# facebookresearch/ProcedureVRL

Measured on AMD Instinct MI355X. Metric: training clips/sec (8f x 224^2, ViT-B TimeSformer), higher is better.
Workload: dtype f16; 1 GPU; TimeSformer ViT-B 8x224^2, 32 clips/GPU, K=9871 step logits, top-5 KL + all-gather InfoNCE, fwd+bwd+AdamW (BASELINE configs[1]; configs[2] at 8 GPUs); clips_per_gpu=32, global_batch=32, parallelism=dp1

## Files before the change

procedurevrl_amd/csrc/attn_bwd_fused.hip:

```cpp
#include "attn_stream.h"
#include "../../include/pvrl.h"

namespace {

constexpr int FB_PRIO7 = 3, FB_PRIO46 = 1;
constexpr int FB_DS = FB_ROWS * 64;
constexpr int FB_Q = 0, FB_D = FB_TILE, FB_K = 2 * FB_TILE, FB_S = 4 * FB_TILE, FB_INIT = 4 * FB_TILE + 2 * FB_DS;
constexpr int FB_O = FB_INIT + 4 * FB_ROWS * 4;
constexpr int FB_LSE = FB_O + 3 * 4096;
constexpr int FB_LDS = FB_LSE + 3 * 256;

struct FbCopy { int o, r0, col; };
__device__ __forceinline__ FbCopy fb_copy_init(int o, int lane) {
  FbCopy cp;
  cp.o = o;
  const int j = o & 3;
  const int band = lane >> 5;
  cp.r0 = 8 * j + 4 * band + ((lane >> 1) & 3);
  const int cb = ((lane >> 3) & 3) ^ band, half = (lane & 1) ^ (j & 1);
  cp.col = 16 * cb + 8 * half;
  if (o >= 12) { cp.r0 = lane & 31; cp.col = 0; }
  return cp;
}
__device__ __forceinline__ void fb_slot_op(const AttnArgs& p, const FbItem& it, int jb, const FbCopy& cp, int rs, int S, unsigned ldsbase) {
  const int rc = min(32 * jb + cp.r0, S - 1);
  const unsigned rowi = rc == 0 ? (unsigned)it.sr.base0 : (unsigned)it.sr.base1 + (unsigned)(rc - 1) * (unsigned)it.sr.stride;
  if (cp.o >= 12) {
    const float* lp = p.lse + ((long)it.seq * p.H + it.h) * S + rc;
    asm volatile("s_mov_b32 m0, %1\n\tglobal_load_lds_dword %0, off" :: "v"(lp), "s"(ldsbase + FB_LSE + rs * 256) : "memory", "m0");
    return;
  }
  const int j = cp.o & 3, typ = cp.o >> 2;
  const int hc = it.h * 64 + cp.col;
  if (typ == 0) {
    glds16_raw_v(p.qkv + (unsigned long long)rowi * (unsigned)p.ld + hc, ldsbase + FB_Q + (4 * jb + j) * 1024);
  } else {
    const op_t* tok = typ == 1 ? p.d_o : p.ofw;
    const op_t* cls = typ == 1 ? p.d_o_cls : p.ofw_cls;
    const op_t* a = tok + (unsigned long long)rowi * (unsigned)p.ldo;
    const op_t* b = cls + (long)it.seq * p.ldo;
    const op_t* src = (p.mp.mode == 1 && rc == 0) ? b : a;
    glds16_raw_v(src + hc, ldsbase + (typ == 1 ? FB_D + (4 * jb + j) * 1024 : FB_O + (4 * rs + j) * 1024));
  }
}
__device__ __forceinline__ void fb_finalize_quarter(const char* smem, int jb, int rs, int qtr, int S, float scale, int lane, float* si) {
  const int pidx = 64 * qtr + lane;
  const int r = pidx >> 3, c8 = (pidx & 7) * 8, row = 32 * jb + r;
  const u32x4 d = *reinterpret_cast<const u32x4*>(smem + FB_D + fb_off(row, c8));
  const u32x4 o = *reinterpret_cast<const u32x4*>(smem + FB_O + rs * 4096 + fb_off(r, c8));
  const float l = reinterpret_cast<const float*>(smem + FB_LSE)[rs * 64 + r];
  float dsum = 0.f;
#pragma unroll
  for (int e = 0; e < 4; ++e) {
    float a0, a1, b0, b1;
    op_unpack2(d[e], a0, a1);
    op_unpack2(o[e], b0, b1);
    dsum = fmaf(a0, b0, dsum);
    dsum = fmaf(a1, b1, dsum);
  }
  dsum = fb_sum8(dsum);
  if ((pidx & 7) == 0) {
    const bool keep = row < S;
    si[row] = keep ? -l * (1.0f / scale) : -INFINITY;
    si[FB_ROWS + row] = keep ? -dsum * scale : 0.f;
  }
}
__device__ __forceinline__ void fb_prime_pair(const AttnArgs& p, const FbItem& it, int pidx, int S, float* si) {
  const int row = pidx >> 3, c8 = (pidx & 7) * 8;
  const int rc = min(row, S - 1);
  const u32x4 d = *reinterpret_cast<const u32x4*>(fb_tok(p.d_o, p.d_o_cls, p.ldo, p, it, rc) + it.h * 64 + c8);
  const u32x4 o = *reinterpret_cast<const u32x4*>(fb_tok(p.ofw, p.ofw_cls, p.ldo, p, it, rc) + it.h * 64 + c8);
  const float l = p.lse[((long)it.seq * p.H + it.h) * S + rc];
  float dsum = 0.f;
#pragma unroll
  for (int e = 0; e < 4; ++e) {
    float a0, a1, b0, b1;
    op_unpack2(d[e], a0, a1);
    op_unpack2(o[e], b0, b1);
    dsum = fmaf(a0, b0, dsum);
    dsum = fmaf(a1, b1, dsum);
  }
  dsum = fb_sum8(dsum);
  if ((pidx & 7) == 0 && row < FB_ROWS) {
    const bool keep = row < S;
    si[row] = keep ? -l / p.scale : -INFINITY;
    si[FB_ROWS + row] = keep ? -dsum * p.scale : 0.f;
  }
}

template <int NQB>
__device__ __forceinline__ void dq_block(const AttnArgs& p, const FbItem& it, const char* Kb, const char* dsr, int nqb, int S,
                                         int jb, int lane) {
  const int g = lane >> 5, hi = (lane >> 4) & 1, i = lane & 15;
  f32x16 acc[2];
#pragma unroll
  for (int dh = 0; dh < 2; ++dh)
#pragma unroll
    for (int r = 0; r < 16; ++r) acc[dh][r] = 0.f;
  const int inb = (i >> 2) * 32 + ((8 * (i & 3)) ^ (16 * g)) + g * 1024;
  const int a0 = inb + hi * 128, a1 = inb + 512 + (hi ^ 1) * 128;
  const int b0 = (2 * g) * 256 + hi * 128 + (i >> 2) * 32 + (((i & 3) ^ (2 * g)) * 8);
  const int b1 = (2 * g + 1) * 256 + hi * 128 + (i >> 2) * 32 + (((i & 3) ^ (2 * g + 1)) * 8);
  auto load = [&](int ks, opx8& bf, opx8* af) {
    bf = tr_frag8(dsr + ks * 1024, b0, b1);
#pragma unroll
    for (int dh = 0; dh < 2; ++dh) af[dh] = tr_frag8(Kb + ks * 2048 + dh * 256, a0, a1);
  };
  if constexpr (NQB > 0) {
    opx8 bf[3], af[3][2];
    load(0, bf[0], af[0]);
    load(1, bf[1], af[1]);
#pragma unroll
    for (int ks = 0; ks < 2 * NQB; ++ks) {
      if (ks + 2 < 2 * NQB) load(ks + 2, bf[(ks + 2) % 3], af[(ks + 2) % 3]);
      __builtin_amdgcn_sched_barrier(0);
#pragma unroll
      for (int dh = 0; dh < 2; ++dh) {
        acc[dh] = MFMA_32x32x16(af[ks % 3][dh], bf[ks % 3], acc[dh], 0, 0, 0);
      }
      __builtin_amdgcn_sched_barrier(0);
    }
  } else {
#pragma unroll 1
    for (int ks = 0; ks < 2 * nqb; ++ks) {
      opx8 bf, af[2];
      load(ks, bf, af);
#pragma unroll
      for (int dh = 0; dh < 2; ++dh) acc[dh] = MFMA_32x32x16(af[dh], bf, acc[dh], 0, 0, 0);
    }
  }
  char* st = const_cast<char*>(dsr);
  {
    const int q = lane & 31;
#pragma unroll
    for (int dh = 0; dh < 2; ++dh)
#pragma unroll
      for (int j = 0; j < 4; ++j) {
        opx4 ov;
#pragma unroll
        for (int r = 0; r < 4; ++r) ov[r] = (op_t)acc[dh][4 * j + r];
        *reinterpret_cast<opx4*>(st + q * 128 + (((4 * dh + j) ^ (q & 7)) * 16) + 8 * g) = ov;
      }
  }
#pragma unroll
  for (int t = 0; t < 4; ++t) {
    const int idx = lane + 64 * t;
    const int r = idx >> 3, ch = idx & 7;
    const u32x4 v = *reinterpret_cast<const u32x4*>(st + r * 128 + ((ch ^ (r & 7)) * 16));
    const int query = 32 * jb + r;
    if (query < S) *reinterpret_cast<u32x4*>(fb_tok(p.dqkv, p.dqkv_cls, p.ldd, p, it, query) + it.h * 64 + ch * 8) = v;
  }
}

template <int NQB>
__global__ __launch_bounds__(512, 2) void attn_bwd_fused_kernel(AttnArgs p, int nvb) {
  __shared__ __attribute__((aligned(16))) char smem[FB_LDS];
  const int tid = threadIdx.x, lane = tid & 63;
  const int wave = __builtin_amdgcn_readfirstlane(tid >> 6);
  const int S = p.mp.S;
  const int nqb = NQB > 0 ? NQB : (S + 31) >> 5;
  const int HD = p.H * PVRL_HEAD_DIM;
  const int n = lane & 31, g = lane >> 5;
  const bool keywave = wave < nqb;
  const float c = p.scale * 1.4426950408889634f;
  const unsigned ldsbase = __builtin_amdgcn_readfirstlane(lds_addr(smem));

  FbItem cur, nxt;
  int vcur = -1;
  int vnxt = fb_next(p, blockIdx.x, gridDim.x, nvb, nxt);
  int par = 0;
  int nit = -1;
  if (vnxt < 0) return;

  {
    float* si = reinterpret_cast<float*>(smem + FB_INIT) + (par ^ 1) * 2 * FB_ROWS;
#pragma unroll
    for (int t = 0; t < 4; ++t) fb_prime_pair(p, nxt, tid + 512 * t, S, si);
  }

  if (wave == 7) {
    __builtin_amdgcn_s_setprio(FB_PRIO7);
    while (true) {
      if (vcur >= 0) {
#pragma unroll 1
        for (int jb = 0; jb < nqb; ++jb) {
          FB_BARRIER();
          dq_block<NQB>(p, cur, smem + FB_K + par * FB_TILE, smem + FB_S + (jb & 1) * FB_DS, nqb, S, jb, lane);
        }
      }
      if (vnxt < 0) break;
      FB_BARRIER();
      par ^= 1; ++nit;
      cur = nxt; vcur = vnxt;
      vnxt = fb_next(p, vcur + gridDim.x, gridDim.x, nvb, nxt);
    }
    return;
  }

  const int rbl = n >> 2, b0 = rbl & 1, b1 = (rbl >> 1) & 1;
  const int rowbase = rbl * 512 + (n & 3) * 32 + ((16 * g) ^ (16 * b1));
  const int e0 = rowbase + b0 * 128, e1 = rowbase + (1 - b0) * 128;
  const int i16 = lane & 15, hi = (lane >> 4) & 1;
  const int trb = g * 512 + (hi ^ g) * 128 + (i16 >> 2) * 32;
  const int tr0 = trb + 8 * (i16 & 3), tr1 = trb + 1024 + ((8 * (i16 & 3)) ^ 16);
  const int kbl = rbl & 3;
  const int dsw0 = (8 * wave + rbl) * 256 + (n & 3) * 32;
  const bool lastkw = wave == nqb - 1 && (S & 31) != 0;
  const float keepf = (32 * wave + n) < S ? 1.f : 0.f;
  const int ncp = wave < 4 ? 3 : (wave == 4 ? 1 : 0);
  const FbCopy cp1 = fb_copy_init(wave < 4 ? wave : 12, lane), cp2 = fb_copy_init(4 + (wave & 3), lane), cp3 = fb_copy_init(8 + (wave & 3), lane);
  if (wave >= 4) __builtin_amdgcn_s_setprio(FB_PRIO46);
  opx8 kf[4], vf[4];
  f32x16 dk[2], dvv[2];
  while (true) {
    opx8 vfn[4];
    if (vnxt >= 0) {
#pragma unroll
      for (int j = 0; j < 4; ++j) {
        const int k = wave + 7 * j;
        int rc, col;
        fb_piece_src(k, lane, S, rc, col);
        glds16_raw_v(p.qkv + row_of(nxt.sr, rc) * p.ld + HD + nxt.h * 64 + col, ldsbase + FB_K + (par ^ 1) * FB_TILE + k * 1024);
      }
      const int key = min(32 * wave + n, S - 1);
      const op_t* vp = p.qkv + row_of(nxt.sr, key) * p.ld + 2 * HD + nxt.h * 64 + 8 * g;
#pragma unroll
      for (int s = 0; s < 4; ++s) vfn[s] = *reinterpret_cast<const opx8*>(vp + 16 * s);
    }

    if (vcur >= 0) {
#pragma unroll
      for (int dh = 0; dh < 2; ++dh)
#pragma unroll
        for (int r = 0; r < 16; ++r) { dk[dh][r] = 0.f; dvv[dh][r] = 0.f; }
      const float* sinit = reinterpret_cast<const float*>(smem + FB_INIT) + par * 2 * FB_ROWS;
      const float* dinit = sinit + FB_ROWS;
#pragma unroll 1
      for (int jb = 0; jb < nqb; ++jb) {
        char* dsj = smem + FB_S + (jb & 1) * FB_DS;
        if (wave < 4) {
          if (jb >= 3) {
            if (vnxt >= 0)
              fb_finalize_quarter(smem, jb - 3, (nqb * nit + jb - 3) % 3, wave, S, p.scale, lane,
                                  reinterpret_cast<float*>(smem + FB_INIT) + (par ^ 1) * 2 * FB_ROWS);
          } else if (jb >= 1 && nit >= 1) {
            fb_finalize_quarter(smem, nqb - 3 + jb, (nqb * (nit - 1) + nqb - 3 + jb) % 3, wave, S, p.scale, lane,
                                reinterpret_cast<float*>(smem + FB_INIT) + par * 2 * FB_ROWS);
          }
        }
        if (keywave) {
          const char* Qj = smem + FB_Q + jb * 4096;
          const char* Dj = smem + FB_D + jb * 4096;
          f32x16 sacc, dacc;
#pragma unroll
          for (int j = 0; j < 4; ++j) {
            const f32x4 a = *reinterpret_cast<const f32x4*>(sinit + 32 * jb + 8 * j + 4 * g);
            const f32x4 b = *reinterpret_cast<const f32x4*>(dinit + 32 * jb + 8 * j + 4 * g);
#pragma unroll
            for (int r = 0; r < 4; ++r) { sacc[4 * j + r] = a[r]; dacc[4 * j + r] = b[r]; }
          }
#pragma unroll
          for (int s = 0; s < 4; ++s) {
            const opx8 qa = *reinterpret_cast<const opx8*>(Qj + ((s & 1) ? e1 : e0) + 256 * (s >> 1));
            sacc = MFMA_32x32x16(qa, kf[s], sacc, 0, 0, 0);
          }
#pragma unroll
          for (int s = 0; s < 4; ++s) {
            const opx8 da = *reinterpret_cast<const opx8*>(Dj + ((s & 1) ? e1 : e0) + 256 * (s >> 1));
            dacc = MFMA_32x32x16(da, vf[s], dacc, 0, 0, 0);
          }
          if (vnxt >= 0 && jb >= 1) {
            const int rs = (nqb * nit + jb - 1) % 3;
            if (ncp >= 1) fb_slot_op(p, nxt, jb - 1, cp1, rs, S, ldsbase);
            if (ncp >= 3) { fb_slot_op(p, nxt, jb - 1, cp2, rs, S, ldsbase); fb_slot_op(p, nxt, jb - 1, cp3, rs, S, ldsbase); }
          }
          opx8 pf[2], sf[2];
#pragma unroll
          for (int r = 0; r < 16; ++r) {
            const float pr = __builtin_amdgcn_exp2f(c * sacc[r]);
            float dsv = pr * dacc[r];
            if (lastkw) dsv *= keepf;
            pf[r >> 3][r & 7] = (op_t)pr;
            sf[r >> 3][r & 7] = (op_t)dsv;
          }
#pragma unroll
          for (int t = 0; t < 2; ++t)
#pragma unroll
            for (int dh = 0; dh < 2; ++dh) {
              const opx8 ad = tr_frag8(Dj + t * 2048 + dh * 256, tr0, tr1);
              dvv[dh] = MFMA_32x32x16(ad, pf[t], dvv[dh], 0, 0, 0);
              const opx8 aq = tr_frag8(Qj + t * 2048 + dh * 256, tr0, tr1);
              dk[dh] = MFMA_32x32x16(aq, sf[t], dk[dh], 0, 0, 0);
            }
#pragma unroll
          for (int j = 0; j < 4; ++j) {
            const int slot = 2 * (j & 1) + g;
            opx4 w;
#pragma unroll
            for (int r = 0; r < 4; ++r) w[r] = sf[j >> 1][4 * (j & 1) + r];
            *reinterpret_cast<opx4*>(dsj + dsw0 + (j >> 1) * 128 + ((slot ^ kbl) * 8)) = w;
          }
        }
        if (!keywave && vnxt >= 0 && jb >= 1) {
          const int rs = (nqb * nit + jb - 1) % 3;
          if (ncp >= 1) fb_slot_op(p, nxt, jb - 1, cp1, rs, S, ldsbase);
          if (ncp >= 3) { fb_slot_op(p, nxt, jb - 1, cp2, rs, S, ldsbase); fb_slot_op(p, nxt, jb - 1, cp3, rs, S, ldsbase); }
        }
        if (ncp >= 3) asm volatile("s_waitcnt vmcnt(3)" ::: "memory");
        else if (ncp >= 1) asm volatile("s_waitcnt vmcnt(1)" ::: "memory");
        else asm volatile("s_waitcnt vmcnt(0)" ::: "memory");
        FB_BARRIER();
      }
      if (wave < 4 && vnxt >= 0)
        fb_finalize_quarter(smem, nqb - 3, (nqb * nit + nqb - 3) % 3, wave, S, p.scale, lane,
                            reinterpret_cast<float*>(smem + FB_INIT) + (par ^ 1) * 2 * FB_ROWS);
      if (vnxt >= 0) {
        const int rs = (nqb * nit + nqb - 1) % 3;
        if (ncp >= 1) fb_slot_op(p, nxt, nqb - 1, cp1, rs, S, ldsbase);
        if (ncp >= 3) { fb_slot_op(p, nxt, nqb - 1, cp2, rs, S, ldsbase); fb_slot_op(p, nxt, nqb - 1, cp3, rs, S, ldsbase); }
      }
    } else {
#pragma unroll 1
      for (int q = 0; q < 8; ++q) fb_slot_op(p, nxt, wave, fb_copy_init(q, lane), 0, S, ldsbase);
      asm volatile("s_waitcnt vmcnt(0)" ::: "memory");
    }

    if (vcur >= 0 && keywave) {
      char* st = smem + FB_S + (nqb & 1) * FB_DS + wave * 2048;
#pragma unroll
      for (int rnd = 0; rnd < 4; ++rnd) {
        const int half = rnd & 1;
        const f32x16* src = (rnd >> 1) ? dvv : dk;
        if ((n >> 4) == half) {
          const int q = n & 15;
#pragma unroll
          for (int dh = 0; dh < 2; ++dh)
#pragma unroll
            for (int j = 0; j < 4; ++j) {
              opx4 ov;
#pragma unroll
              for (int r = 0; r < 4; ++r) ov[r] = (op_t)src[dh][4 * j + r];
              *reinterpret_cast<opx4*>(st + q * 128 + (((4 * dh + j) ^ (q & 7)) * 16) + 8 * g) = ov;
            }
        }
        asm volatile("" ::: "memory");
#pragma unroll
        for (int t = 0; t < 2; ++t) {
          const int idx = lane + 64 * t;
          const int r = idx >> 3, ch = idx & 7;
          const u32x4 v = *reinterpret_cast<const u32x4*>(st + r * 128 + ((ch ^ (r & 7)) * 16));
          const int key = 32 * wave + 16 * half + r;
          if (key < S)
            *reinterpret_cast<u32x4*>(fb_tok(p.dqkv, p.dqkv_cls, p.ldd, p, cur, key) + ((rnd >> 1) ? 2 * HD : HD) + cur.h * 64 + ch * 8) = v;
        }
      }
    }
    if (vnxt < 0) break;
    FB_BARRIER();
    par ^= 1; ++nit;
    cur = nxt; vcur = vnxt;
    vnxt = fb_next(p, vcur + gridDim.x, gridDim.x, nvb, nxt);
    {
      const char* Kc = smem + FB_K + par * FB_TILE + wave * 4096;
#pragma unroll
      for (int s = 0; s < 4; ++s) {
        kf[s] = *reinterpret_cast<const opx8*>(Kc + ((s & 1) ? e1 : e0) + 256 * (s >> 1));
#pragma unroll
        for (int e = 0; e < 8; ++e) vf[s][e] = (op_t)((float)vfn[s][e] * p.scale);
      }
    }
  }
}

}

bool pvrl_attn_bwd_fused_ok(const AttnArgs& p) {
  if (p.causal || p.kpm) return false;
  if (p.mp.S <= 96 || p.mp.S > FB_ROWS) return false;
  if ((long)p.nseq * p.mp.S >= (1L << 31)) return false;
  if ((p.ldd % 8) || (p.ldo % 8)) return false;
  int e = 0;
  const float m = frexpf(p.scale, &e);
  return m == 0.5f;
}

int pvrl_attn_bwd_fused_launch(const AttnArgs& p, hipStream_t s) {
  const int cus = 8 * pvrl_compute_cus_per_xcd();
  const int nvb = 8 * ((p.nseq + 7) / 8) * p.H;
  const int grid = nvb < cus ? nvb : cus;
  if (p.mp.S > 192) hipLaunchKernelGGL(attn_bwd_fused_kernel<7>, dim3(grid), dim3(512), 0, s, p, nvb);
  else hipLaunchKernelGGL(attn_bwd_fused_kernel<0>, dim3(grid), dim3(512), 0, s, p, nvb);
  PVRL_LAUNCH_CHECK();
  return PVRL_OK;
}
```

procedurevrl_amd/csrc/attn_mfma.hip:

```cpp
#include "attn_common.h"
#include "../../include/pvrl.h"

bool pvrl_attn_bwd_fused_ok(const AttnArgs& p);
int pvrl_attn_bwd_fused_launch(const AttnArgs& p, hipStream_t s);
bool pvrl_attn_bwd_s32_ok(const AttnArgs& p);
int pvrl_attn_bwd_s32_launch(const AttnArgs& p, hipStream_t s);

namespace {

template <int NKT, bool GEN>
__device__ __forceinline__ unsigned long long pad_bits_q(const AttnArgs& p, int seq, int q4) {
  unsigned long long bits = 0ull;
  if constexpr (GEN) {
    if (p.kpm) {
#pragma unroll
      for (int kt = 0; kt < NKT; ++kt)
#pragma unroll
        for (int r = 0; r < 4; ++r) {
          const int key = kt * 16 + 4 * q4 + r;
          if (key < p.mp.S && p.kpm[(long)seq * p.mp.S + key]) bits |= 1ull << (kt * 4 + r);
        }
    }
  }
  return bits;
}

template <int NT, int ROWS = ATT_ROWS_PAD>
struct TileRegs { u32x4 v[(ROWS * 8 + NT - 1) / NT]; };

template <int NT, int ROWS = ATT_ROWS_PAD>
__device__ __forceinline__ void tile_issue(TileRegs<NT, ROWS>& t, const op_t* base, long ld, int col0, const SeqRows& sr, int S,
                                           const op_t* src0, int rows, int tid) {
  constexpr int ITERS = (ROWS * 8 + NT - 1) / NT;
#pragma unroll
  for (int it = 0; it < ITERS; ++it) {
    const int idx = tid + NT * it;
    const int row = idx >> 3, c = idx & 7;
    const int rc = min(row, S - 1);
    const op_t* src = (rc == 0 && src0) ? src0 : base + row_of(sr, rc) * ld;
    const u32x4 v = *reinterpret_cast<const u32x4*>(src + col0 + c * 8);
    const unsigned keep = row < S ? 0xffffffffu : 0u;
    t.v[it] = v & (u32x4){keep, keep, keep, keep};
    (void)rows;
  }
}
template <int NT, int ROWS = ATT_ROWS_PAD>
__device__ __forceinline__ void tile_commit(const TileRegs<NT, ROWS>& t, char* bl, int rows, int tid) {
  constexpr int ITERS = (ROWS * 8 + NT - 1) / NT;
#pragma unroll
  for (int it = 0; it < ITERS; ++it) {
    const int idx = tid + NT * it;
    const int row = idx >> 3, c = idx & 7;
    if (row < rows) *reinterpret_cast<u32x4*>(bl + bl_off(row, c * 8)) = t.v[it];
  }
}

template <int NKT, bool GEN, int NW, int SC = 0>
__global__ __launch_bounds__(64 * NW, NKT > 13 ? 2 : (NW + 1) / 2) void attn_fwd_kernel(AttnArgs p) {
  constexpr int NKS2 = (NKT + 1) / 2;
  constexpr int BL = NKS2 * 32 * 128;
  __shared__ __attribute__((aligned(16))) char smem[2 * BL];
  char* Kb = smem;
  char* Vb = smem + BL;
  const int tid = threadIdx.x, lane = tid & 63;
  const int wave = __builtin_amdgcn_readfirstlane(tid >> 6);
  const int xj = blockIdx.x >> 3;
  const int seq = (xj / p.H) * 8 + (blockIdx.x & 7), h = xj % p.H;
  if (seq >= p.nseq) return;
  const int S = SC ? SC : p.mp.S;
  const int HD = p.H * PVRL_HEAD_DIM;
  const SeqRows sr = seq_rows(p.mp, seq);
  constexpr int MAXT = (NKT + NW - 1) / NW;
  const int q4 = lane >> 4, i = lane & 15;
  const int nqt = (S + 15) >> 4;
  opx8 qf[MAXT][2];
#pragma unroll
  for (int t = 0; t < MAXT; ++t) {
    const int query = (wave + t * NW) * 16 + i;
    const int qrow = query < S ? query : S - 1;
    const op_t* qp = p.qkv + row_of(sr, qrow) * p.ld + h * 64 + q4 * 8;
    qf[t][0] = *reinterpret_cast<const opx8*>(qp);
    qf[t][1] = *reinterpret_cast<const opx8*>(qp + 32);
  }
  {
    TileRegs<64 * NW, NKS2 * 32> kr, vr;
    tile_issue<64 * NW, NKS2 * 32>(kr, p.qkv, p.ld, HD + h * 64, sr, S, nullptr, NKS2 * 32, tid);
    tile_issue<64 * NW, NKS2 * 32>(vr, p.qkv, p.ld, 2 * HD + h * 64, sr, S, nullptr, NKS2 * 32, tid);
    tile_commit<64 * NW, NKS2 * 32>(kr, Kb, NKS2 * 32, tid);
    tile_commit<64 * NW, NKS2 * 32>(vr, Vb, NKS2 * 32, tid);
  }
  __syncthreads();

  const unsigned long long pbits = pad_bits_q<NKT, GEN>(p, seq, q4);
#pragma unroll
  for (int t = 0; t < MAXT; ++t) {
    const int qt = wave + t * NW;
    if (qt >= nqt) break;
    const int query = qt * 16 + i;
    const opx8 qf0 = qf[t][0], qf1 = qf[t][1];

    f32x4 sc[NKT];
#pragma unroll
    for (int kt = 0; kt < NKT; ++kt) {
      const int krow = kt * 16 + i;
      const opx8 k0 = bl_row_frag(Kb, krow, q4);
      const opx8 k1 = bl_row_frag(Kb, krow, 4 + q4);
      f32x4 a = (f32x4){0.f, 0.f, 0.f, 0.f};
      a = MFMA_16x16x32(k0, qf0, a, 0, 0, 0);
      sc[kt] = MFMA_16x16x32(k1, qf1, a, 0, 0, 0);
      if (NKT > 5 && (kt & 1)) __builtin_amdgcn_sched_barrier(0);
    }
    const float c = p.scale * 1.4426950408889634f;
    float mx = -INFINITY;
#pragma unroll
    for (int kt = 0; kt < NKT; ++kt)
#pragma unroll
      for (int r = 0; r < 4; ++r) {
        const int key = kt * 16 + 4 * q4 + r;
        if (GEN || kt * 16 + 15 >= S) {
          bool msk = key >= S;
          if constexpr (GEN) msk = msk || ((pbits >> (kt * 4 + r)) & 1ull) || (p.causal && key > query);
          if (msk) sc[kt][r] = -INFINITY;
        }
        mx = fmaxf(mx, sc[kt][r]);
      }
    mx = fmaxf(mx, __shfl_xor(mx, 16, 64));
    mx = fmaxf(mx, __shfl_xor(mx, 32, 64));
    const float mref = (mx == -INFINITY) ? 0.f : mx;
    const float mc = mref * c;
    float sum = 0.f;
#pragma unroll
    for (int kt = 0; kt < NKT; ++kt)
#pragma unroll
      for (int r = 0; r < 4; ++r) {
        const float e = __builtin_amdgcn_exp2f(fmaf(sc[kt][r], c, -mc));
        sc[kt][r] = e;
        sum += e;
      }
    sum += __shfl_xor(sum, 16, 64);
    sum += __shfl_xor(sum, 32, 64);
    const float inv = sum > 0.f ? 1.0f / sum : 0.f;

    f32x4 oacc[4];
#pragma unroll
    for (int dt = 0; dt < 4; ++dt) oacc[dt] = (f32x4){0.f, 0.f, 0.f, 0.f};
#pragma unroll
    for (int ks2 = 0; ks2 < NKS2; ++ks2) {
      opx8 pf;
#pragma unroll
      for (int r = 0; r < 4; ++r) {
        pf[r] = (op_t)sc[2 * ks2][r];
        if (2 * ks2 + 1 < NKT) pf[4 + r] = (op_t)sc[(2 * ks2 + 1 < NKT) ? 2 * ks2 + 1 : 0][r];
        else pf[4 + r] = (op_t)0.f;
      }
#pragma unroll
      for (int dt = 0; dt < 4; ++dt) {
        const opx8 vf = bl_frag(Vb, ks2, dt, lane);
        oacc[dt] = MFMA_16x16x32(vf, pf, oacc[dt], 0, 0, 0);
      }
      if (NKT > 5) __builtin_amdgcn_sched_barrier(0);
    }
    if (query < S) {
      op_t* op = tok_ptr(p.o, p.o_cls, p.ldo, p.mp, sr, seq, query) + h * 64 + 4 * q4;
#pragma unroll
      for (int dt = 0; dt < 4; ++dt) {
        opx4 ov;
#pragma unroll
        for (int r = 0; r < 4; ++r) ov[r] = (op_t)(oacc[dt][r] * inv);
        *reinterpret_cast<opx4*>(op + 16 * dt) = ov;
      }
      if (q4 == 0 && p.lse) p.lse[((long)seq * p.H + h) * S + query] = mref * p.scale + __logf(sum);
    }
  }
}

template <int NKT, bool GEN, int NW, int SC = 0>
__global__ __launch_bounds__(64 * NW, NKT > 13 ? 2 : (NW + 1) / 2) void attn_bwd_q_kernel(AttnArgs p) {
  constexpr int NKS2 = (NKT + 1) / 2;
  constexpr int BL = NKS2 * 32 * 128;
  __shared__ __attribute__((aligned(16))) char smem[2 * BL];
  char* Kb = smem;
  char* Vb = smem + BL;
  const int tid = threadIdx.x, lane = tid & 63;
  const int wave = __builtin_amdgcn_readfirstlane(tid >> 6);
  const int xj = blockIdx.x >> 3;
  const int seq = (xj / p.H) * 8 + (blockIdx.x & 7), h = xj % p.H;
  if (seq >= p.nseq) return;
  const int S = SC ? SC : p.mp.S;
  const int HD = p.H * PVRL_HEAD_DIM;
  const SeqRows sr = seq_rows(p.mp, seq);
  constexpr int MAXT = (NKT + NW - 1) / NW;
  const int q4 = lane >> 4, i = lane & 15;
  const int nqt = (S + 15) >> 4;
  const float c = p.scale * 1.4426950408889634f;
  opx8 qf[MAXT][2], df[MAXT][2];
  float lse2[MAXT], dss[MAXT];
  {
    opx8 of[MAXT][2];
#pragma unroll
    for (int t = 0; t < MAXT; ++t) {
      const int query = (wave + t * NW) * 16 + i;
      const int qj = query < S ? query : S - 1;
      const op_t* qp = p.qkv + row_of(sr, qj) * p.ld + h * 64 + q4 * 8;
      qf[t][0] = *reinterpret_cast<const opx8*>(qp);
      qf[t][1] = *reinterpret_cast<const opx8*>(qp + 32);
      const op_t* dop = tok_ptr(p.d_o, p.d_o_cls, p.ldo, p.mp, sr, seq, qj) + h * 64 + q4 * 8;
      df[t][0] = *reinterpret_cast<const opx8*>(dop);
      df[t][1] = *reinterpret_cast<const opx8*>(dop + 32);
      const op_t* ofp = tok_ptr(p.ofw, p.ofw_cls, p.ldo, p.mp, sr, seq, qj) + h * 64 + q4 * 8;
      of[t][0] = *reinterpret_cast<const opx8*>(ofp);
      of[t][1] = *reinterpret_cast<const opx8*>(ofp + 32);
      lse2[t] = p.lse[((long)seq * p.H + h) * S + qj] * 1.4426950408889634f;
    }
    TileRegs<64 * NW, NKS2 * 32> kr, vr;
    tile_issue<64 * NW, NKS2 * 32>(kr, p.qkv, p.ld, HD + h * 64, sr, S, nullptr, NKS2 * 32, tid);
    tile_issue<64 * NW, NKS2 * 32>(vr, p.qkv, p.ld, 2 * HD + h * 64, sr, S, nullptr, NKS2 * 32, tid);
#pragma unroll
    for (int t = 0; t < MAXT; ++t) {
      float dsum = 0.f;
#pragma unroll
      for (int e = 0; e < 8; ++e) dsum += (float)df[t][0][e] * (float)of[t][0][e] + (float)df[t][1][e] * (float)of[t][1][e];
      dsum += __shfl_xor(dsum, 16, 64);
      dsum += __shfl_xor(dsum, 32, 64);
      dss[t] = dsum * p.scale;
      const int query = (wave + t * NW) * 16 + i;
      if (q4 == 0 && query < S) p.dvec[((long)seq * p.H + h) * S + query] = dsum;
    }
    tile_commit<64 * NW, NKS2 * 32>(kr, Kb, NKS2 * 32, tid);
    tile_commit<64 * NW, NKS2 * 32>(vr, Vb, NKS2 * 32, tid);
  }
  __syncthreads();

  const unsigned long long pbits = pad_bits_q<NKT, GEN>(p, seq, q4);
#pragma unroll
  for (int t = 0; t < MAXT; ++t) {
    const int qt = wave + t * NW;
    if (qt >= nqt) break;
    const int query = qt * 16 + i;
    const opx8 qf0 = qf[t][0], qf1 = qf[t][1], df0 = df[t][0], df1 = df[t][1];
    const float lse2_t = lse2[t], dss_t = dss[t];

    f32x4 dq[4];
#pragma unroll
    for (int dt = 0; dt < 4; ++dt) dq[dt] = (f32x4){0.f, 0.f, 0.f, 0.f};
#pragma unroll
    for (int ks2 = 0; ks2 < NKS2; ++ks2) {
      opx8 sf;
#pragma unroll
      for (int half = 0; half < 2; ++half) {
        const int kt = 2 * ks2 + half;
        if (kt >= NKT) {
#pragma unroll
          for (int r = 0; r < 4; ++r) sf[4 * half + r] = (op_t)0.f;
          continue;
        }
        const int krow = kt * 16 + i;
        const opx8 k0 = bl_row_frag(Kb, krow, q4);
        const opx8 k1 = bl_row_frag(Kb, krow, 4 + q4);
        const opx8 v0 = bl_row_frag(Vb, krow, q4);
        const opx8 v1 = bl_row_frag(Vb, krow, 4 + q4);
        f32x4 s = (f32x4){0.f, 0.f, 0.f, 0.f};
        s = MFMA_16x16x32(k0, qf0, s, 0, 0, 0);
        s = MFMA_16x16x32(k1, qf1, s, 0, 0, 0);
        f32x4 dp = (f32x4){0.f, 0.f, 0.f, 0.f};
        dp = MFMA_16x16x32(v0, df0, dp, 0, 0, 0);
        dp = MFMA_16x16x32(v1, df1, dp, 0, 0, 0);
#pragma unroll
        for (int r = 0; r < 4; ++r) {
          const int key = kt * 16 + 4 * q4 + r;
          float pr = __builtin_amdgcn_exp2f(fmaf(s[r], c, -lse2_t));
          if (GEN || kt * 16 + 15 >= S) {
            bool msk = key >= S || (GEN && query >= S);
            if constexpr (GEN) msk = msk || ((pbits >> (kt * 4 + r)) & 1ull) || (p.causal && key > query);
            if (msk) pr = 0.f;
          }
          sf[4 * half + r] = (op_t)(pr * fmaf(dp[r], p.scale, -dss_t));
        }
      }
#pragma unroll
      for (int dt = 0; dt < 4; ++dt) {
        const opx8 kf = bl_frag(Kb, ks2, dt, lane);
        dq[dt] = MFMA_16x16x32(kf, sf, dq[dt], 0, 0, 0);
      }
      if (NKT > 5) __builtin_amdgcn_sched_barrier(0);
    }
    if (query < S) {
      op_t* op = tok_ptr(p.dqkv, p.dqkv_cls, p.ldd, p.mp, sr, seq, query) + h * 64 + 4 * q4;
#pragma unroll
      for (int dt = 0; dt < 4; ++dt) {
        opx4 ov;
#pragma unroll
        for (int r = 0; r < 4; ++r) ov[r] = (op_t)dq[dt][r];
        *reinterpret_cast<opx4*>(op + 16 * dt) = ov;
      }
    }
  }
}

template <int NKT, bool GEN, int NW, int SC = 0>
__global__ __launch_bounds__(64 * NW, NKT > 13 ? 2 : (NW + 1) / 2) void attn_bwd_kv_kernel(AttnArgs p) {
  constexpr int NKS2 = (NKT + 1) / 2;
  constexpr int ROWS = NKS2 * 32;
  constexpr int T = ROWS * 128;
  __shared__ __attribute__((aligned(16))) char smem[2 * T + 2 * ROWS * 4];
  char* Qb = smem;
  char* Db = smem + T;
  float* lse_s = reinterpret_cast<float*>(smem + 2 * T);
  float* dv_s = lse_s + ROWS;
  const int tid = threadIdx.x, lane = tid & 63;
  const int wave = __builtin_amdgcn_readfirstlane(tid >> 6);
  const int xj = blockIdx.x >> 3;
  const int seq = (xj / p.H) * 8 + (blockIdx.x & 7), h = xj % p.H;
  if (seq >= p.nseq) return;
  const int S = SC ? SC : p.mp.S;
  const int HD = p.H * PVRL_HEAD_DIM;
  const SeqRows sr = seq_rows(p.mp, seq);
  constexpr int MAXT = (NKT + NW - 1) / NW;
  const int q4 = lane >> 4, i = lane & 15;
  const float c = p.scale * 1.4426950408889634f;
  const int nkt_rt = (S + 15) >> 4;
  opx8 kf[MAXT][2], vf[MAXT][2];
#pragma unroll
  for (int t = 0; t < MAXT; ++t) {
    const int key = (wave + t * NW) * 16 + i;
    const int kj = key < S ? key : S - 1;
    const op_t* kp = p.qkv + row_of(sr, kj) * p.ld + HD + h * 64 + q4 * 8;
    kf[t][0] = *reinterpret_cast<const opx8*>(kp);
    kf[t][1] = *reinterpret_cast<const opx8*>(kp + 32);
    vf[t][0] = *reinterpret_cast<const opx8*>(kp + HD);
    vf[t][1] = *reinterpret_cast<const opx8*>(kp + HD + 32);
  }
  {
    const op_t* src0 = p.mp.mode == 1 ? p.d_o_cls + (long)seq * p.ldo : nullptr;
    TileRegs<64 * NW, ROWS> qr, dr;
    tile_issue<64 * NW, ROWS>(qr, p.qkv, p.ld, h * 64, sr, S, nullptr, ROWS, tid);
    tile_issue<64 * NW, ROWS>(dr, p.d_o, p.ldo, h * 64, sr, S, src0, ROWS, tid);
    for (int idx = tid; idx < ROWS; idx += 64 * NW) {
      const long stat = ((long)seq * p.H + h) * S + idx;
      lse_s[idx] = idx < S ? p.lse[stat] * 1.4426950408889634f : 0.f;
      dv_s[idx] = idx < S ? p.dvec[stat] * p.scale : 0.f;
    }
    tile_commit<64 * NW, ROWS>(qr, Qb, ROWS, tid);
    tile_commit<64 * NW, ROWS>(dr, Db, ROWS, tid);
  }
  __syncthreads();

#pragma unroll
  for (int t = 0; t < MAXT; ++t) {
    const int kt = wave + t * NW;
    if (kt >= nkt_rt) break;
    const int key = kt * 16 + i;
    const int kj = key < S ? key : S - 1;
    const opx8 kf0 = kf[t][0], kf1 = kf[t][1], vf0 = vf[t][0], vf1 = vf[t][1];
    bool kbad = key >= S;
    if constexpr (GEN) kbad = kbad || (p.kpm ? (p.kpm[(long)seq * S + kj] != 0) : false);

    f32x4 dk[4], dv[4];
#pragma unroll
    for (int dt = 0; dt < 4; ++dt) { dk[dt] = (f32x4){0.f, 0.f, 0.f, 0.f}; dv[dt] = (f32x4){0.f, 0.f, 0.f, 0.f}; }

#pragma unroll 1
    for (int u = 0; u < NKS2; ++u) {
      opx8 pf, sf;
#pragma unroll
      for (int half = 0; half < 2; ++half) {
        const int qrow = (2 * u + half) * 16 + i;
        const opx8 a0 = bl_row_frag(Qb, qrow, q4);
        const opx8 a1 = bl_row_frag(Qb, qrow, 4 + q4);
        const opx8 d0 = bl_row_frag(Db, qrow, q4);
        const opx8 d1 = bl_row_frag(Db, qrow, 4 + q4);
        f32x4 s = (f32x4){0.f, 0.f, 0.f, 0.f};
        s = MFMA_16x16x32(a0, kf0, s, 0, 0, 0);
        s = MFMA_16x16x32(a1, kf1, s, 0, 0, 0);
        f32x4 dp = (f32x4){0.f, 0.f, 0.f, 0.f};
        dp = MFMA_16x16x32(d0, vf0, dp, 0, 0, 0);
        dp = MFMA_16x16x32(d1, vf1, dp, 0, 0, 0);
        const int qb = (2 * u + half) * 16 + 4 * q4;
        const f32x4 l4 = *reinterpret_cast<const f32x4*>(lse_s + qb);
        const f32x4 d4 = *reinterpret_cast<const f32x4*>(dv_s + qb);
#pragma unroll
        for (int r = 0; r < 4; ++r) {
          const int query = qb + r;
          bool msk = query >= S || kbad;
          if constexpr (GEN) msk = msk || (p.causal && key > query);
          const float pr = msk ? 0.f : __builtin_amdgcn_exp2f(fmaf(s[r], c, -l4[r]));
          pf[half * 4 + r] = (op_t)pr;
          sf[half * 4 + r] = (op_t)(pr * fmaf(dp[r], p.scale, -d4[r]));
        }
      }
#pragma unroll
      for (int dt = 0; dt < 4; ++dt) {
        const opx8 qtf = bl_frag(Qb, u, dt, lane);
        const opx8 dtf = bl_frag(Db, u, dt, lane);
        dk[dt] = MFMA_16x16x32(qtf, sf, dk[dt], 0, 0, 0);
        dv[dt] = MFMA_16x16x32(dtf, pf, dv[dt], 0, 0, 0);
      }
    }
    if (key < S) {
      op_t* op = tok_ptr(p.dqkv, p.dqkv_cls, p.ldd, p.mp, sr, seq, key) + HD + h * 64 + 4 * q4;
#pragma unroll
      for (int dt = 0; dt < 4; ++dt) {
        opx4 ok, ov;
#pragma unroll
        for (int r = 0; r < 4; ++r) { ok[r] = (op_t)dk[dt][r]; ov[r] = (op_t)dv[dt][r]; }
        *reinterpret_cast<opx4*>(op + 16 * dt) = ok;
        *reinterpret_cast<opx4*>(op + HD + 16 * dt) = ov;
      }
    }
  }
}

int check_common(const AttnArgs& p) {
  if (!p.qkv || p.H <= 0 || p.nseq < 0 || p.mp.S <= 0 || p.mp.S > ATT_ROWS_LONG) return PVRL_EINVAL;
  if ((p.ld % 8)) return PVRL_EINVAL;
  if (p.mp.mode == 1 && (p.mp.T <= 0 || (p.nseq % p.mp.T))) return PVRL_EINVAL;
  if ((p.causal || p.kpm) && p.mp.S > ATT_ROWS) return PVRL_EINVAL;
  return PVRL_OK;
}

template <int NKT, int NW>
int launch_fwd(const AttnArgs& p, hipStream_t s) {
  const dim3 grid((unsigned)(8 * ((p.nseq + 7) / 8) * p.H)), blk(64 * NW);
  constexpr int SFIX = NKT == 13 ? 197 : NKT == 2 ? 32 : 0;
  if (p.causal || p.kpm) hipLaunchKernelGGL((attn_fwd_kernel<NKT, true, NW>), grid, blk, 0, s, p);
  else if (SFIX && p.mp.S == SFIX) hipLaunchKernelGGL((attn_fwd_kernel<NKT, false, NW, SFIX>), grid, blk, 0, s, p);
  else hipLaunchKernelGGL((attn_fwd_kernel<NKT, false, NW>), grid, blk, 0, s, p);
  PVRL_LAUNCH_CHECK();
  return PVRL_OK;
}

template <int NKT, int NW>
int launch_bwd(const AttnArgs& p, hipStream_t s) {
  const dim3 grid((unsigned)(8 * ((p.nseq + 7) / 8) * p.H)), blk(64 * NW);
  constexpr int SFIX = NKT == 13 ? 197 : NKT == 2 ? 32 : 0;
  if (p.causal || p.kpm) {
    hipLaunchKernelGGL((attn_bwd_q_kernel<NKT, true, NW>), grid, blk, 0, s, p);
    PVRL_LAUNCH_CHECK();
    hipLaunchKernelGGL((attn_bwd_kv_kernel<NKT, true, NW>), grid, blk, 0, s, p);
  } else if (SFIX && p.mp.S == SFIX) {
    hipLaunchKernelGGL((attn_bwd_q_kernel<NKT, false, NW, SFIX>), grid, blk, 0, s, p);
    PVRL_LAUNCH_CHECK();
    hipLaunchKernelGGL((attn_bwd_kv_kernel<NKT, false, NW, SFIX>), grid, blk, 0, s, p);
  } else {
    hipLaunchKernelGGL((attn_bwd_q_kernel<NKT, false, NW>), grid, blk, 0, s, p);
    PVRL_LAUNCH_CHECK();
    hipLaunchKernelGGL((attn_bwd_kv_kernel<NKT, false, NW>), grid, blk, 0, s, p);
  }
  PVRL_LAUNCH_CHECK();
  return PVRL_OK;
}

}

extern "C" int pvrl_attn_fwd(const void* qkv, int64_t ld, int64_t nseq, int64_t S, int64_t H, int mode, int64_t T,
                             int64_t cls_base, float scale, int causal, const void* key_padding_mask, void* o,
                             void* o_cls, int64_t ldo, float* lse, void* stream) {
  AttnArgs p = {};
  p.qkv = (const op_t*)qkv; p.ld = ld; p.H = (int)H; p.nseq = (int)nseq;
  p.mp.mode = mode; p.mp.S = (int)S; p.mp.T = (int)T; p.mp.cls_base = cls_base;
  p.scale = scale; p.causal = causal; p.kpm = (const unsigned char*)key_padding_mask;
  p.o = (op_t*)o; p.o_cls = (op_t*)o_cls; p.ldo = ldo; p.lse = lse;
  if (nseq == 0) return PVRL_OK;
  if (int e = check_common(p)) return e;
  if (!o || (ldo % 4) || (mode == 1 && !o_cls)) return PVRL_EINVAL;
  hipStream_t s = (hipStream_t)stream;
  if (S <= 16) return launch_fwd<1, 4>(p, s);
  if (S <= 32) return launch_fwd<2, 4>(p, s);
  if (S <= 48) return launch_fwd<3, 4>(p, s);
  if (S <= 80) return launch_fwd<5, 4>(p, s);
  if (S <= 208) return launch_fwd<13, 8>(p, s);
  if (S <= 272) return launch_fwd<17, 8>(p, s);
  return launch_fwd<26, 8>(p, s);
}

extern "C" int pvrl_attn_bwd(const void* qkv, int64_t ld, int64_t nseq, int64_t S, int64_t H, int mode, int64_t T,
                             int64_t cls_base, float scale, int causal, const void* key_padding_mask, const void* o,
                             const void* o_cls, const void* d_o, const void* d_o_cls, int64_t ldo, const float* lse,
                             float* dvec, void* dqkv, void* dqkv_cls, int64_t ldd, void* stream) {
  AttnArgs p = {};
  p.qkv = (const op_t*)qkv; p.ld = ld; p.H = (int)H; p.nseq = (int)nseq;
  p.mp.mode = mode; p.mp.S = (int)S; p.mp.T = (int)T; p.mp.cls_base = cls_base;
  p.scale = scale; p.causal = causal; p.kpm = (const unsigned char*)key_padding_mask;
  p.ofw = (const op_t*)o; p.ofw_cls = (const op_t*)o_cls; p.d_o = (const op_t*)d_o; p.d_o_cls = (const op_t*)d_o_cls;
  p.ldo = ldo; p.lse = const_cast<float*>(lse); p.dvec = dvec;
  p.dqkv = (op_t*)dqkv; p.dqkv_cls = (op_t*)dqkv_cls; p.ldd = ldd;
  if (nseq == 0) return PVRL_OK;
  if (int e = check_common(p)) return e;
  if (!o || !d_o || !lse || !dvec || !dqkv || (ldo % 8) || (ldd % 4)) return PVRL_EINVAL;
  if (mode == 1 && (!o_cls || !d_o_cls || !dqkv_cls)) return PVRL_EINVAL;
  hipStream_t s = (hipStream_t)stream;
  if (pvrl_attn_bwd_fused_ok(p)) return pvrl_attn_bwd_fused_launch(p, s);
  if (pvrl_attn_bwd_s32_ok(p)) return pvrl_attn_bwd_s32_launch(p, s);
  if (S <= 16) return launch_bwd<1, 4>(p, s);
  if (S <= 32) return launch_bwd<2, 4>(p, s);
  if (S <= 48) return launch_bwd<3, 4>(p, s);
  if (S <= 80) return launch_bwd<5, 4>(p, s);
  if (S <= 208) return launch_bwd<13, 8>(p, s);
  if (S <= 272) return launch_bwd<17, 8>(p, s);
  return launch_bwd<26, 8>(p, s);
}
```

Measured before the change: 725.7 clips/s.

## Add 32-row-tile forward attention kernel for S=197 and backward ablation switches

Adds a new forward attention kernel for the spatial S=197 case. It stages the whole K and V image in LDS, processes 32-query tiles with 32x32x16 MFMAs in a single-pass softmax, and stages the output through LDS for coalesced 16-byte stores. The kernel is dispatched when the output pointers and stride are aligned. It also adds compile-time ablation flags to the fused backward kernel (default off) and a probe guard around the extern entry points. The new kernel trades register pressure, since it holds all score tiles, and higher LDS use for less online-softmax rescaling and better store coalescing.

```diff
diff --git a/procedurevrl_amd/csrc/attn_bwd_fused.hip b/procedurevrl_amd/csrc/attn_bwd_fused.hip
--- a/procedurevrl_amd/csrc/attn_bwd_fused.hip
+++ b/procedurevrl_amd/csrc/attn_bwd_fused.hip
@@ -1,7 +1,17 @@
 #include "attn_stream.h"
 #include "../../include/pvrl.h"
 
+#ifndef PVRL_FB_ABLATE
+#define PVRL_FB_ABLATE 0
+#endif
+
 namespace {
+
+__device__ __forceinline__ void fb_keep(const opx8& v) {
+  union { opx8 v; u32x4 u; } x;
+  x.v = v;
+  asm volatile("" :: "v"(x.u[0]), "v"(x.u[1]), "v"(x.u[2]), "v"(x.u[3]));
+}
 
 constexpr int FB_PRIO7 = 3, FB_PRIO46 = 1;
 constexpr int FB_DS = FB_ROWS * 64;
@@ -152,8 +162,9 @@
   }
 }
 
-template <int NQB>
+template <int NQB, int ABL = PVRL_FB_ABLATE>
 __global__ __launch_bounds__(512, 2) void attn_bwd_fused_kernel(AttnArgs p, int nvb) {
+  constexpr bool A_STREAM = ABL & 17, A_DQ = ABL & 18, A_EXP = ABL & 4, A_DKV = ABL & 8, A_ALL = ABL & 16;
   __shared__ __attribute__((aligned(16))) char smem[FB_LDS];
   const int tid = threadIdx.x, lane = tid & 63;
   const int wave = __builtin_amdgcn_readfirstlane(tid >> 6);
@@ -185,7 +196,7 @@
 #pragma unroll 1
         for (int jb = 0; jb < nqb; ++jb) {
           FB_BARRIER();
-          dq_block<NQB>(p, cur, smem + FB_K + par * FB_TILE, smem + FB_S + (jb & 1) * FB_DS, nqb, S, jb, lane);
+          if constexpr (!A_DQ) dq_block<NQB>(p, cur, smem + FB_K + par * FB_TILE, smem + FB_S + (jb & 1) * FB_DS, nqb, S, jb, lane);
         }
       }
       if (vnxt < 0) break;
@@ -214,7 +225,13 @@
   f32x16 dk[2], dvv[2];
   while (true) {
     opx8 vfn[4];
-    if (vnxt >= 0) {
+    if constexpr (A_STREAM) {
+#pragma unroll
+      for (int s = 0; s < 4; ++s)
+#pragma unroll
+        for (int e = 0; e < 8; ++e) vfn[s][e] = (op_t)0.f;
+    }
+    if (!A_STREAM && vnxt >= 0) {
 #pragma unroll
       for (int j = 0; j < 4; ++j) {
         const int k = wave + 7 * j;
@@ -238,7 +255,7 @@
 #pragma unroll 1
       for (int jb = 0; jb < nqb; ++jb) {
         char* dsj = smem + FB_S + (jb & 1) * FB_DS;
-        if (wave < 4) {
+        if (!A_ALL && wave < 4) {
           if (jb >= 3) {
             if (vnxt >= 0)
               fb_finalize_quarter(smem, jb - 3, (nqb * nit + jb - 3) % 3, wave, S, p.scale, lane,
@@ -248,7 +265,7 @@
                                 reinterpret_cast<float*>(smem + FB_INIT) + par * 2 * FB_ROWS);
           }
         }
-        if (keywave) {
+        if (!A_ALL && keywave) {
           const char* Qj = smem + FB_Q + jb * 4096;
           const char* Dj = smem + FB_D + jb * 4096;
           f32x16 sacc, dacc;
@@ -269,7 +286,7 @@
             const opx8 da = *reinterpret_cast<const opx8*>(Dj + ((s & 1) ? e1 : e0) + 256 * (s >> 1));
             dacc = MFMA_32x32x16(da, vf[s], dacc, 0, 0, 0);
           }
-          if (vnxt >= 0 && jb >= 1) {
+          if (!A_STREAM && vnxt >= 0 && jb >= 1) {
             const int rs = (nqb * nit + jb - 1) % 3;
             if (ncp >= 1) fb_slot_op(p, nxt, jb - 1, cp1, rs, S, ldsbase);
             if (ncp >= 3) { fb_slot_op(p, nxt, jb - 1, cp2, rs, S, ldsbase); fb_slot_op(p, nxt, jb - 1, cp3, rs, S, ldsbase); }
@@ -277,14 +294,15 @@
           opx8 pf[2], sf[2];
 #pragma unroll
           for (int r = 0; r < 16; ++r) {
-            const float pr = __builtin_amdgcn_exp2f(c * sacc[r]);
-            float dsv = pr * dacc[r];
-            if (lastkw) dsv *= keepf;
+            const float pr = A_EXP ? sacc[r] : __builtin_amdgcn_exp2f(c * sacc[r]);
+            float dsv = A_EXP ? dacc[r] : pr * dacc[r];
+            if (!A_EXP && lastkw) dsv *= keepf;
             pf[r >> 3][r & 7] = (op_t)pr;
             sf[r >> 3][r & 7] = (op_t)dsv;
           }
-#pragma unroll
-          for (int t = 0; t < 2; ++t)
+          if constexpr (A_DKV) { fb_keep(pf[0]); fb_keep(pf[1]); fb_keep(sf[0]); fb_keep(sf[1]); }
+#pragma unroll
+          for (int t = 0; t < (A_DKV ? 0 : 2); ++t)
 #pragma unroll
             for (int dh = 0; dh < 2; ++dh) {
               const opx8 ad = tr_frag8(Dj + t * 2048 + dh * 256, tr0, tr1);
@@ -293,7 +311,7 @@
               dk[dh] = MFMA_32x32x16(aq, sf[t], dk[dh], 0, 0, 0);
             }
 #pragma unroll
-          for (int j = 0; j < 4; ++j) {
+          for (int j = 0; j < (A_DQ ? 0 : 4); ++j) {
             const int slot = 2 * (j & 1) + g;
             opx4 w;
 #pragma unroll
@@ -301,7 +319,7 @@
             *reinterpret_cast<opx4*>(dsj + dsw0 + (j >> 1) * 128 + ((slot ^ kbl) * 8)) = w;
           }
         }
-        if (!keywave && vnxt >= 0 && jb >= 1) {
+        if (!A_STREAM && !keywave && vnxt >= 0 && jb >= 1) {
           const int rs = (nqb * nit + jb - 1) % 3;
           if (ncp >= 1) fb_slot_op(p, nxt, jb - 1, cp1, rs, S, ldsbase);
           if (ncp >= 3) { fb_slot_op(p, nxt, jb - 1, cp2, rs, S, ldsbase); fb_slot_op(p, nxt, jb - 1, cp3, rs, S, ldsbase); }
@@ -311,10 +329,10 @@
         else asm volatile("s_waitcnt vmcnt(0)" ::: "memory");
         FB_BARRIER();
       }
-      if (wave < 4 && vnxt >= 0)
+      if (!A_ALL && wave < 4 && vnxt >= 0)
         fb_finalize_quarter(smem, nqb - 3, (nqb * nit + nqb - 3) % 3, wave, S, p.scale, lane,
                             reinterpret_cast<float*>(smem + FB_INIT) + (par ^ 1) * 2 * FB_ROWS);
-      if (vnxt >= 0) {
+      if (!A_STREAM && vnxt >= 0) {
         const int rs = (nqb * nit + nqb - 1) % 3;
         if (ncp >= 1) fb_slot_op(p, nxt, nqb - 1, cp1, rs, S, ldsbase);
         if (ncp >= 3) { fb_slot_op(p, nxt, nqb - 1, cp2, rs, S, ldsbase); fb_slot_op(p, nxt, nqb - 1, cp3, rs, S, ldsbase); }
@@ -325,7 +343,7 @@
       asm volatile("s_waitcnt vmcnt(0)" ::: "memory");
     }
 
-    if (vcur >= 0 && keywave) {
+    if (!A_ALL && vcur >= 0 && keywave) {
       char* st = smem + FB_S + (nqb & 1) * FB_DS + wave * 2048;
 #pragma unroll
       for (int rnd = 0; rnd < 4; ++rnd) {
diff --git a/procedurevrl_amd/csrc/attn_mfma.hip b/procedurevrl_amd/csrc/attn_mfma.hip
--- a/procedurevrl_amd/csrc/attn_mfma.hip
+++ b/procedurevrl_amd/csrc/attn_mfma.hip
@@ -1,4 +1,4 @@
-#include "attn_common.h"
+#include "attn_stream.h"
 #include "../../include/pvrl.h"
 
 bool pvrl_attn_bwd_fused_ok(const AttnArgs& p);
@@ -170,6 +170,169 @@
         *reinterpret_cast<opx4*>(op + 16 * dt) = ov;
       }
       if (q4 == 0 && p.lse) p.lse[((long)seq * p.H + h) * S + query] = mref * p.scale + __logf(sum);
+    }
+  }
+}
+
+template <int SC, int NW, int OCC, bool STAGE>
+__global__ __launch_bounds__(64 * NW, (NW * OCC + 3) / 4) void attn_fwd32_kernel(AttnArgs p) {
+  static_assert(SC > 192 && SC <= 208, "7 query tiles of 32, 13 key steps of 16");
+  constexpr int S = SC, NQT = 7, ROWS = 208, IMG = ROWS * 128, NT = 64 * NW;
+  constexpr int MAXT = (NQT + NW - 1) / NW;
+  constexpr int ITERS = (ROWS * 8 + NT - 1) / NT;
+  static_assert(!STAGE || NQT * 4096 <= 2 * IMG, "the output stage lives in the dead images");
+  __shared__ __attribute__((aligned(16))) char smem[2 * IMG];
+  char* Kb = smem;
+  char* Vb = smem + IMG;
+  const int tid = threadIdx.x, lane = tid & 63;
+  const int wave = __builtin_amdgcn_readfirstlane(tid >> 6);
+  const int xj = blockIdx.x >> 3;
+  const int seq = (xj / p.H) * 8 + (blockIdx.x & 7), h = xj % p.H;
+  if (seq >= p.nseq) return;
+  const int HD = p.H * PVRL_HEAD_DIM;
+  const SeqRows sr = seq_rows(p.mp, seq);
+  const int n = lane & 31, g = lane >> 5;
+  opx8 qf[4];
+  auto load_q = [&](int qt) {
+    const int query = min(qt * 32 + n, S - 1);
+    const op_t* qp = p.qkv + row_of(sr, query) * p.ld + h * 64 + 8 * g;
+#pragma unroll
+    for (int s = 0; s < 4; ++s) qf[s] = *reinterpret_cast<const opx8*>(qp + 16 * s);
+  };
+  load_q(wave);
+  {
+    u32x4 kr[ITERS], vr[ITERS];
+#pragma unroll
+    for (int it = 0; it < ITERS; ++it) {
+      const int idx = tid + NT * it;
+      const int row = idx >> 3, c = idx & 7;
+      const op_t* src = p.qkv + row_of(sr, min(row, S - 1)) * p.ld + HD + h * 64 + c * 8;
+      const unsigned keep = row < S ? 0xffffffffu : 0u;
+      kr[it] = *reinterpret_cast<const u32x4*>(src) & (u32x4){keep, keep, keep, keep};
+      vr[it] = *reinterpret_cast<const u32x4*>(src + HD) & (u32x4){keep, keep, keep, keep};
+    }
+#pragma unroll
+    for (int it = 0; it < ITERS; ++it) {
+      const int idx = tid + NT * it;
+      const int row = idx >> 3, c = idx & 7;
+      if (row < ROWS) {
+        *reinterpret_cast<u32x4*>(Kb + fb_off(row, c * 8)) = kr[it];
+        *reinterpret_cast<u32x4*>(Vb + fb_off(row, c * 8)) = vr[it];
+      }
+    }
+  }
+  __syncthreads();
+
+  const int i16 = lane & 15, hi = (lane >> 4) & 1;
+  const int trb = g * 512 + (hi ^ g) * 128 + (i16 >> 2) * 32;
+  const int tr0 = trb + 8 * (i16 & 3), tr1 = trb + 1024 + ((8 * (i16 & 3)) ^ 16);
+  const float c = p.scale * 1.4426950408889634f;
+  unsigned opk[MAXT][16];
+#pragma unroll
+  for (int t = 0; t < MAXT; ++t) {
+    const int qt = wave + t * NW;
+    if (qt >= NQT) break;
+    const int query = qt * 32 + n;
+
+    f32x16 sc[NQT];
+#pragma unroll
+    for (int kt = 0; kt < NQT; ++kt) {
+      const int krow = min(kt * 32 + n, ROWS - 1);
+#pragma unroll
+      for (int r = 0; r < 16; ++r) sc[kt][r] = 0.f;
+#pragma unroll
+      for (int s = 0; s < 4; ++s) {
+        const opx8 ka = *reinterpret_cast<const opx8*>(Kb + fb_off(krow, 16 * s + 8 * g));
+        sc[kt] = MFMA_32x32x16(ka, qf[s], sc[kt], 0, 0, 0);
+      }
+      __builtin_amdgcn_sched_barrier(0);
+    }
+    float mx = -INFINITY;
+#pragma unroll
+    for (int kt = 0; kt < NQT; ++kt)
+#pragma unroll
+      for (int r = 0; r < 16; ++r) {
+        const int key = kt * 32 + 8 * (r >> 2) + 4 * g + (r & 3);
+        if (kt * 32 + 31 >= S && key >= S) sc[kt][r] = -INFINITY;
+        mx = fmaxf(mx, sc[kt][r]);
+      }
+    mx = fmaxf(mx, __shfl_xor(mx, 32, 64));
+    const float mc = mx * c;
+    float sum = 0.f;
+    unsigned pk[NQT][8];
+#pragma unroll
+    for (int kt = 0; kt < NQT; ++kt)
+#pragma unroll
+      for (int r = 0; r < 16; r += 2) {
+        const float e0 = __builtin_amdgcn_exp2f(fmaf(sc[kt][r], c, -mc));
+        const float e1 = __builtin_amdgcn_exp2f(fmaf(sc[kt][r + 1], c, -mc));
+        pk[kt][r >> 1] = pack_opx2(e0, e1);
+        sum += e0;
+        sum += e1;
+      }
+    sum += __shfl_xor(sum, 32, 64);
+    if (t + 1 < MAXT) load_q(qt + NW);
+    const float inv = 1.0f / sum;
+
+    f32x16 oacc[2];
+#pragma unroll
+    for (int dh = 0; dh < 2; ++dh)
+#pragma unroll
+      for (int r = 0; r < 16; ++r) oacc[dh][r] = 0.f;
+#pragma unroll
+    for (int ks = 0; ks < ROWS / 16; ++ks) {
+      union { u32x4 u; opx8 v; } pfu;
+#pragma unroll
+      for (int e = 0; e < 4; ++e) pfu.u[e] = pk[ks >> 1][4 * (ks & 1) + e];
+      const opx8 pf = pfu.v;
+#pragma unroll
+      for (int dh = 0; dh < 2; ++dh) {
+        const opx8 va = tr_frag8(Vb + ks * 2048 + dh * 256, tr0, tr1);
+        oacc[dh] = MFMA_32x32x16(va, pf, oacc[dh], 0, 0, 0);
+      }
+    }
+    if (g == 0 && query < S && p.lse) p.lse[((long)seq * p.H + h) * S + query] = mx * p.scale + __logf(sum);
+    if constexpr (STAGE) {
+#pragma unroll
+      for (int dh = 0; dh < 2; ++dh)
+#pragma unroll
+        for (int j = 0; j < 4; ++j) {
+          opk[t][8 * dh + 2 * j] = pack_opx2(oacc[dh][4 * j] * inv, oacc[dh][4 * j + 1] * inv);
+          opk[t][8 * dh + 2 * j + 1] = pack_opx2(oacc[dh][4 * j + 2] * inv, oacc[dh][4 * j + 3] * inv);
+        }
+#pragma unroll
+      for (int e = 0; e < 16; ++e) asm volatile("" : "+v"(opk[t][e]));
+    } else if (query < S) {
+      op_t* op = tok_ptr(p.o, p.o_cls, p.ldo, p.mp, sr, seq, query) + h * 64 + 4 * g;
+#pragma unroll
+      for (int dh = 0; dh < 2; ++dh)
+#pragma unroll
+        for (int j = 0; j < 4; ++j) {
+          opx4 ov;
+#pragma unroll
+          for (int r = 0; r < 4; ++r) ov[r] = (op_t)(oacc[dh][4 * j + r] * inv);
+          *reinterpret_cast<opx4*>(op + 32 * dh + 8 * j) = ov;
+        }
+    }
+  }
+  if constexpr (STAGE) {
+    __syncthreads();
+#pragma unroll
+    for (int t = 0; t < MAXT; ++t) {
+      const int qt = wave + t * NW;
+      if (qt >= NQT) break;
+      char* st = smem + qt * 4096;
+#pragma unroll
+      for (int ch = 0; ch < 8; ++ch)
+        *reinterpret_cast<u32x2*>(st + n * 128 + ((ch ^ (n & 7)) * 16) + 8 * g) = (u32x2){opk[t][2 * ch], opk[t][2 * ch + 1]};
+#pragma unroll
+      for (int u = 0; u < 4; ++u) {
+        const int idx = lane + 64 * u;
+        const int r = idx >> 3, ch = idx & 7;
+        const u32x4 v = *reinterpret_cast<const u32x4*>(st + r * 128 + ((ch ^ (r & 7)) * 16));
+        const int query = 32 * qt + r;
+        if (query < S) *reinterpret_cast<u32x4*>(tok_ptr(p.o, p.o_cls, p.ldo, p.mp, sr, seq, query) + h * 64 + ch * 8) = v;
+      }
     }
   }
 }
@@ -418,11 +581,17 @@
   return PVRL_OK;
 }
 
+bool fwd32_rows_ok(const AttnArgs& p) {
+  return (p.ldo % 8) == 0 && ((uintptr_t)p.o % 16) == 0 && ((uintptr_t)p.o_cls % 16) == 0;
+}
+
 template <int NKT, int NW>
 int launch_fwd(const AttnArgs& p, hipStream_t s) {
   const dim3 grid((unsigned)(8 * ((p.nseq + 7) / 8) * p.H)), blk(64 * NW);
   constexpr int SFIX = NKT == 13 ? 197 : NKT == 2 ? 32 : 0;
   if (p.causal || p.kpm) hipLaunchKernelGGL((attn_fwd_kernel<NKT, true, NW>), grid, blk, 0, s, p);
+  else if (SFIX == 197 && p.mp.S == SFIX && fwd32_rows_ok(p))
+    hipLaunchKernelGGL((attn_fwd32_kernel<(SFIX == 197 ? SFIX : 197), 4, 3, true>), grid, dim3(256), 0, s, p);
   else if (SFIX && p.mp.S == SFIX) hipLaunchKernelGGL((attn_fwd_kernel<NKT, false, NW, SFIX>), grid, blk, 0, s, p);
   else hipLaunchKernelGGL((attn_fwd_kernel<NKT, false, NW>), grid, blk, 0, s, p);
   PVRL_LAUNCH_CHECK();
@@ -452,6 +621,7 @@
 
 }
 
+#ifndef PVRL_ATTN_PROBE
 extern "C" int pvrl_attn_fwd(const void* qkv, int64_t ld, int64_t nseq, int64_t S, int64_t H, int mode, int64_t T,
                              int64_t cls_base, float scale, int causal, const void* key_padding_mask, void* o,
                              void* o_cls, int64_t ldo, float* lse, void* stream) {
@@ -499,3 +669,4 @@
   if (S <= 272) return launch_bwd<17, 8>(p, s);
   return launch_bwd<26, 8>(p, s);
 }
+#endif
```

After: 727.5 clips/s, median of 6. About the same (+0.2%).
